# YuvalNirkin/hyperseg

Measured on AMD Instinct MI355X. Metric: frames/sec @ bs=1 HyperSeg-M 1024x512, higher is better.
Workload: dtype f32 storage and accumulation; level-4 inverted residual products as 3-term f16 splits (f32-class: 1.3e-7 of sum|a||b|; exact_f32 beside it)

## Files before the change

### hyperseg_amd/_hip.py

```python
import ctypes as C
import os

import torch

_LIB_PATH = os.environ.get('HS_HIP_LIB') or os.path.join(os.path.dirname(os.path.abspath(__file__)), 'lib',
                                                         'libhyperseg_hip.so')

ACT_NONE, ACT_RELU, ACT_RELU6, ACT_SWISH = 0, 1, 2, 3
PAD_MODES = {'zeros': 0, 'reflect': 1, 'replicate': 2, 'circular': 3}
PREV_NONE, PREV_SAME, PREV_BILINEAR = 0, 1, 2

_STATUS = {-1: 'bad argument', -2: 'feature map does not tile into the weight grid (H % fh or W % fw != 0)',
           -3: 'unsupported shape', -4: 'tile does not fit the LDS'}


class HipLibraryError(RuntimeError):
    pass


class StageInputC(C.Structure):
    _fields_ = [('skip', C.c_void_p), ('prev', C.c_void_p),
                ('batch', C.c_int32), ('H', C.c_int32), ('W', C.c_int32),
                ('c_skip', C.c_int32), ('c_prev', C.c_int32),
                ('Hp', C.c_int32), ('Wp', C.c_int32),
# ... 130 lines not shown
        'hs_mbconv_expand_dw_se_fwd': ([vp, i32, i32, i32, i32, vp, i32, vp, vp, vp, i32, i32, i32, i32, i32, i32, vp, vp, vp, C.POINTER(SeTailC), vp], C.c_int),
        'hs_se_tail_workspace': ([i32, i32, i32, i32, i64], C.c_int64),
        'hs_se_tail_tails': ([i32, i32, i32, i64], C.c_int),
        'hs_mbconv_se_workgroups': ([i32, i32, i32, i32, i32, i32], C.c_int64),
        'hs_stem_conv_fwd': ([vp, i32, i32, i32, i32, vp, i32, i32, i32, i32, i32, vp, vp, vp, vp], C.c_int),
        'hs_mbconv_tiles': ([i32, i32, i32, i32], C.c_int),
        'hs_stem_dw_fwd': ([vp, i32, i32, i32, vp, i32, vp, vp, i32, i32, i32, i32, vp, i32, i32, i32, vp, vp, vp, vp, vp], C.c_int),
        'hs_image_ingest_fwd': ([vp, i32, i32, i32, i32, i32, vp, vp, vp], C.c_int),
        'hs_stem_dw_u8_fwd': ([vp, i32, vp, i32, i32, i32, vp, i32, vp, vp, i32, i32, i32, i32, vp, i32, i32, i32, vp, vp, vp, vp, vp], C.c_int),
        'hs_overlay_fwd': ([vp, vp, i32, i32, i32, i32, vp, i32, i32, vp, vp], C.c_int),
        'hs_upsample_overlay_fwd': ([vp, i32, i32, i32, i32, i32, i32, vp, i32, vp, i32, i32, vp, vp, vp], C.c_int),
        'hs_mbconv_expand_dw_fwd': ([vp, i32, i32, i32, i32, vp, i32, vp, vp, vp, i32, i32, i32, i32, i32, i32, vp, vp, vp, vp, vp], C.c_int),
        'hs_se_gate_fwd': ([vp, i32, i32, i32, C.c_float, vp, vp, i32, vp, vp, vp, vp, vp, i32, vp, vp, vp], C.c_int),
        'hs_gemm_split_kp': ([i32], C.c_int),
        'hs_gemm_split_fwd': ([vp, vp, vp, vp, vp, i32, vp, vp, i32, i32, i32, i32, i32, vp], C.c_int),
        'hs_gemm_split_conv2x2_fwd': ([vp, vp, vp, vp, i32, vp, vp, i32, i32, i32, i32, i32, i32, vp], C.c_int),
        'hs_gemm_split_up2_fwd': ([vp, vp, vp, vp, i32, vp, i32, i32, i32, i32, i32, i32, vp], C.c_int),
        'hs_pooled_shift_fwd': ([vp, i32, C.c_float, vp, vp, vp, i32, i32, vp], C.c_int),
    }
    for name, (argtypes, restype) in sig.items():
        fn = getattr(lib, name)
        fn.argtypes, fn.restype = argtypes, restype
    if lib.hs_version() != 1:
        raise HipLibraryError(f'ABI mismatch: library reports version {lib.hs_version()}, binding expects 1')
    return lib


lib = _load()
EXPORTS = ['hs_version', 'hs_build_info', 'hs_signal2weights_fwd', 'hs_signal2weights_multi_fwd', 'hs_s2w_pack_floats', 'hs_s2w_pack_fwd', 'hs_bank_pack_fwd', 'hs_bn_fold_fwd',
           'hs_patch_conv_fwd', 'hs_patch_conv_s2w_fwd', 'hs_k1_chain_workspace', 'hs_k1_chain_fwd', 'hs_decoder_chain_workspace', 'hs_decoder_chain_fwd', 'hs_meta_conv_fwd', 'hs_meta_conv_bwd', 'hs_patch_conv_gen_fwd', 'hs_patch_ir_fwd', 'hs_patch_ir_v0_fwd', 'hs_patch_ir_v0_ws_fwd', 'hs_patch_ir_v0_workspace', 'hs_patch_ir_route', 'hs_ir_tile_map', 'hs_upsample_bilinear_fwd', 'hs_upsample_argmax_fwd',
           'hs_stage_input_fwd', 'hs_depthwise_conv_fwd', 'hs_depthwise_pool_blocks', 'hs_stem_conv_fwd', 'hs_stem_dw_fwd', 'hs_mbconv_tiles', 'hs_mbconv_expand_dw_fwd', 'hs_se_gate_fwd', 'hs_depthwise_conv_se_fwd', 'hs_mbconv_expand_dw_se_fwd', 'hs_se_tail_workspace', 'hs_se_tail_tails', 'hs_mbconv_se_workgroups', 'hs_pointwise_conv_fwd', 'hs_affine_act_fwd', 'hs_gemm_split_kp', 'hs_gemm_split_fwd', 'hs_gemm_split_conv2x2_fwd', 'hs_gemm_split_up2_fwd', 'hs_pooled_shift_fwd', 'hs_patch_conv_bwd_input',
           'hs_patch_conv_bwd_weight', 'hs_halo_tiles_fwd', 'hs_halo_tiles_bwd', 'hs_tile_interior_fwd', 'hs_tile_interior_bwd', 'hs_dw_tiles_fwd', 'hs_dw_tiles_bwd_in', 'hs_dw_tiles_bwd_w',
           'hs_s2w_train_fwd', 'hs_s2w_train_workspace', 'hs_s2w_train_bwd', 'hs_cross_entropy_fwd', 'hs_cross_entropy_bwd', 'hs_cross_entropy_typed_fwd', 'hs_cross_entropy_typed_bwd', 'hs_bootstrapped_ce_fwd', 'hs_bootstrapped_ce_bwd', 'hs_bootstrap_mean_workspace', 'hs_bootstrap_mean_fwd', 'hs_bootstrap_mean_bwd', 'hs_bootstrap_mean_batched_fwd', 'hs_bootstrap_mean_batched_bwd', 'hs_bn_train_workspace', 'hs_bn_train_stats_fwd', 'hs_dw_tiles_bn_fwd', 'hs_dw_tiles_bn_bwd_w', 'hs_patch_conv_bn_fwd', 'hs_patch_conv_bn_bwd_w', 'hs_adam_blocks', 'hs_adam_step', 'hs_bootstrap_mean_of_batch_fwd', 'hs_bootstrap_mean_of_batch_bwd', 'hs_upsample_bilinear_bwd', 'hs_upsample_bilinear_typed_bwd', 'hs_upsample_bilinear_bf16_fwd', 'hs_stage_input_typed_fwd', 'hs_bank_unpack_fwd', 'hs_bn_act_train_fwd',
           'hs_bn_act_train_bwd', 'hs_dw_tiles_bn_bwd_in_partials', 'hs_dw_tiles_bn_bwd_in', 'hs_bn_act_train_bwd_apply', 'hs_patch_conv_plain_fwd', 'hs_patch_conv_plain_bwd_in', 'hs_patch_conv_plain_bwd_w',
           'hs_upsample_bilinear_f16_fwd', 'hs_adam_step_amp', 'hs_eval_max_classes', 'hs_upsample_confusion_fwd', 'hs_confusion_fwd',
           'hs_image_ingest_fwd', 'hs_stem_dw_u8_fwd', 'hs_overlay_fwd', 'hs_upsample_overlay_fwd']


def check(status, what):
    if status == 0:
        return
    if status < 0:
        raise HipLibraryError(f'{what}: {_STATUS.get(status, status)}')
    raise HipLibraryError(f'{what}: HIP launch failed with hipError_t {status}')


# ... 35 lines not shown
```

### hyperseg_amd/csrc/hs_gemm_split.hip

```cpp
#include "hs_common.h"
#include <type_traits>

namespace hs {

using half8 = __attribute__((ext_vector_type(8))) _Float16;
using gs_f32x4 = __attribute__((ext_vector_type(4))) float;

__device__ __forceinline__ int gs_exp_of(float m) { return min(max(__float_as_int(m) >> 23, 27), 254); }
__device__ __forceinline__ float gs_scale_of(int eb) { return __int_as_float((268 - eb) << 23); }
__device__ __forceinline__ float gs_inv_scale_of(int eb) { return __int_as_float((eb - 14) << 23); }

struct GemmSplitArgs {
    const _Float16* __restrict__ wf;
    const float* __restrict__ w_inv;
    const float* __restrict__ gate; const float* __restrict__ x;
    const float* shift;
    const float* residual;
    float* y;
    int M, K, KST, N, act;
    int conv_wo;
    float* pool_partial;
    int up2_wo;
};

// ... 248 lines not shown
        ps_mean[c] = t * inv_p;
    }
    __syncthreads();
    const int r0 = 16 * blockIdx.x + 4 * wave;
    float acc[4] = {0.f, 0.f, 0.f, 0.f};
#pragma unroll 2
    for (int c = lane; c < C; c += 64) {
        const float m = ps_mean[c];
#pragma unroll
        for (int i = 0; i < 4; ++i) acc[i] = fmaf(wb[(size_t)min(r0 + i, M - 1) * C + c], m, acc[i]);
    }
#pragma unroll
    for (int i = 0; i < 4; ++i) {
        const float t = wave_sum64(acc[i]);
        if (lane == 0 && r0 + i < M) out[r0 + i] = shift[r0 + i] + t;
    }
}

static bool gemm_split_plan(int K, int& nwv, int& ks, int& nch) {
    const int steps = (K + 31) / 32;
    nwv = 2;
    while (nwv < 8 && nwv < steps) nwv *= 2;
    const int per = (steps + nwv - 1) / nwv;
    nch = per > 5 ? 2 : 1;
    ks = (steps + nwv * nch - 1) / (nwv * nch);
    return ks <= 5;
}

}

// ... 90 lines not shown
#define HS_GP(KSV, NCHV) hipLaunchKernelGGL((gemm_split_kernel<KSV, 8, true, 1, 2, NCHV, true>), grid, dim3(512), lds, s, a)
    switch (ks * 2 + nch - 1) {
        case 2: HS_GP(1, 1); break;
        case 4: HS_GP(2, 1); break;
        case 6: HS_GP(3, 1); break;
        case 8: HS_GP(4, 1); break;
        case 10: HS_GP(5, 1); break;
        case 7: HS_GP(3, 2); break;
        case 9: HS_GP(4, 2); break;
        case 11: HS_GP(5, 2); break;
        default: return HS_ERR_UNSUPPORTED;
    }
#undef HS_GP
    return launch_status();
}
```

### hyperseg_amd/functional.py

```python
import ctypes as C
import functools
import os
import threading

import torch

from . import _hip
from ._hip import ACT_NONE, ACT_RELU, ACT_RELU6, PAD_MODES

BN_EPS_DEFAULT = 1e-5
S2W_TRAIN_MAX_LAYERS = 8
COSCHEDULE_BANKS = os.environ.get('HS_COSCHEDULE_BANKS', '0') == '1'


def _round_up(n, m):
    return (n + m - 1) // m * m


def _device_of(a):
    if isinstance(a, torch.Tensor):
        return a.device
    if isinstance(a, (StageInput, BankRef, SignalRef, U8Frame)):
        return a.device
    return None
# ... 989 lines not shown
    if residual is not None and tuple(residual.shape) != shape:
        raise ValueError(f'residual has shape {tuple(residual.shape)}, expected {shape}')
    if gate is not None and tuple(gate.shape) != (b, cin):
        raise ValueError(f'gate has shape {tuple(gate.shape)}, expected {(b, cin)}')
    if shift is not None and shift.numel() != sw.c_out:
        raise ValueError(f'shift has {shift.numel()} entries, expected {sw.c_out}')
    st = _hip.lib.hs_gemm_split_fwd(_hip.dev_ptr(sw.frag, 'w_frag', torch.float16), _hip.dev_ptr(sw.inv, 'w_inv'),
                                    _hip.dev_ptr(gate, 'gate') if gate is not None else None, _hip.dev_ptr(x, 'x'),
                                    _hip.dev_ptr(shift, 'shift') if shift is not None else None, int(act),
                                    _hip.dev_ptr(residual, 'residual') if residual is not None else None,
                                    _hip.dev_ptr(out, 'out'), b, sw.c_out, cin, sw.kp, h * w, _hip.stream_ptr())
    _hip.check(st, 'hs_gemm_split_fwd')
    return out


@_on_operand_device
def gemm_split_conv2x2(sw, x, shift=None, act=ACT_NONE, out=None, pool_partial=None):
    b, cin, h, w = x.shape
    if 4 * cin != sw.c_in:
        raise ValueError(f'input has {cin} channels, the weight {sw.c_in} / 4')
    if h % 2 or w % 4:
        raise ValueError(f'map {h}x{w}: height must be even and width a multiple of 4')
    shape = (b, sw.c_out, h // 2, w // 2)
    if out is None:
        out = torch.empty(shape, device=x.device, dtype=torch.float32)
    elif tuple(out.shape) != shape:
        raise ValueError(f'out has shape {tuple(out.shape)}, expected {shape}')
    if shift is not None and shift.numel() != sw.c_out:
        raise ValueError(f'shift has {shift.numel()} entries, expected {sw.c_out}')
    nblk = -(-(h // 2) * (w // 2) // 16)
# ... 249 lines not shown
```

### hyperseg_amd/models/backbones/efficientnet.py

```python
import math
from functools import partial

import torch
import torch.nn as nn
import torch.nn.functional as F

_B0_STAGES = [
    (1, 3, 1, 32, 16, 1),
    (6, 3, 2, 16, 24, 2),
    (6, 5, 2, 24, 40, 2),
    (6, 3, 2, 40, 80, 3),
    (6, 5, 1, 80, 112, 3),
    (6, 5, 2, 112, 192, 4),
    (6, 3, 1, 192, 320, 1),
]
_SCALING = {
    'efficientnet-b0': (1.0, 1.0, 224, 0.2), 'efficientnet-b1': (1.0, 1.1, 240, 0.2),
    'efficientnet-b2': (1.1, 1.2, 260, 0.3), 'efficientnet-b3': (1.2, 1.4, 300, 0.3),
    'efficientnet-b4': (1.4, 1.8, 380, 0.4), 'efficientnet-b5': (1.6, 2.2, 456, 0.4),
    'efficientnet-b6': (1.8, 2.6, 528, 0.5), 'efficientnet-b7': (2.0, 3.1, 600, 0.5),
}
_BN_MOMENTUM, _BN_EPS, _SE_RATIO, _DIVISOR = 0.01, 1e-3, 0.25, 8


# ... 46 lines not shown
        self.stride, self.in_f, self.out_f, self.expand = stride, in_f, out_f, expand
        mid = in_f * expand
        bn = partial(nn.BatchNorm2d, momentum=_BN_MOMENTUM, eps=_BN_EPS)
        if expand != 1:
            self._expand_conv = SamePadConv2d(in_f, mid, 1, image_size=image_size, bias=False)
            self._bn0 = bn(mid)
        self._depthwise_conv = SamePadConv2d(mid, mid, kernel, stride, image_size=image_size, groups=mid, bias=False)
        self._bn1 = bn(mid)
        squeezed = max(1, int(in_f * _SE_RATIO))
        self._se_reduce = SamePadConv2d(mid, squeezed, 1, image_size=1)
        self._se_expand = SamePadConv2d(squeezed, mid, 1, image_size=1)
        self._project_conv = SamePadConv2d(mid, out_f, 1, image_size=_out_size(image_size, stride), bias=False)
        self._bn2 = bn(out_f)
        self._fused_dw = None
        self._fused_active = None

    def forward(self, inputs, drop_connect_rate=None):
        active = self._fused_active if self._fused_active is not None else _inference_only(self, inputs)
        if self._fused_dw is not None and active:
            return self._fused_dw(inputs, self)
        x = inputs
        if self.expand != 1:
            x = F.silu(self._bn0(self._expand_conv(x)))
        x = F.silu(self._bn1(self._depthwise_conv(x)))
        gate = self._se_expand(F.silu(self._se_reduce(F.adaptive_avg_pool2d(x, 1))))
        x = self._bn2(self._project_conv(torch.sigmoid(gate) * x))
        if self.stride == 1 and self.in_f == self.out_f:
            if drop_connect_rate and self.training:
                keep = 1.0 - drop_connect_rate
                mask = torch.floor(keep + torch.rand(x.shape[0], 1, 1, 1, dtype=x.dtype, device=x.device))
# ... 64 lines not shown
            return False
        h, w = (inputs.shape[2] + 1) // 2, (inputs.shape[3] + 1) // 2
        for blk in self._blocks:
            st = blk._depthwise_conv.stride[0]
            if (h * w) % 4 != 0:
                return False
            h, w = (h + st - 1) // st, (w + st - 1) // st
        return (h * w) % 4 == 0

    def takes_u8_frame(self, frame):
        f0 = self._blocks[0]._fused_dw if len(self._blocks) else None
        return self._fused_stem is not None and f0 is not None and f0.takes_image() and self._fused_ok(frame)

    def extract_features_list(self, inputs):
        use = self._fused_ok(inputs)
        for blk in self._blocks:
            blk._fused_active = use
        try:
            return self._extract_features_list(inputs, use)
        finally:
            for blk in self._blocks:
                blk._fused_active = None

    def _extract_features_list(self, inputs, use):
        f0 = self._blocks[0]._fused_dw if len(self._blocks) else None
        if self._fused_stem is not None and use and f0 is not None and getattr(f0, '_stem', None) is not None:
            x = inputs
        elif self._fused_stem is not None and use:
            x = self._fused_stem(inputs)
        else:
            x = F.silu(self._bn0(self._conv_stem(inputs)))
        feats = []
        n = len(self._blocks)
        for idx, block in enumerate(self._blocks):
            rate = self.drop_connect_rate * float(idx) / n if self.drop_connect_rate else None
            x = block(x, drop_connect_rate=rate)
            if self._res_feat_mask[idx]:
# ... 26 lines not shown
```

### hyperseg_amd/utils/inference.py

```python
import contextlib
import os

import torch
import torch.nn as nn


class InputNorm:

    LAYOUTS = ('hwc', 'chw')

    def __init__(self, mean=(0.485, 0.456, 0.406), std=(0.229, 0.224, 0.225), layout='hwc'):
        if layout not in self.LAYOUTS:
            raise ValueError(f'layout {layout!r}: expected one of {self.LAYOUTS}')
        self.mean = torch.as_tensor(mean, dtype=torch.float32).flatten().clone()
        self.std = torch.as_tensor(std, dtype=torch.float32).flatten().clone()
        if self.mean.numel() != 3 or self.std.numel() != 3:
            raise ValueError('mean and std must hold one value per channel of a 3-channel frame')
        if bool((self.std == 0).any()):
            raise ValueError('std must be non-zero')
        self.layout = layout
        values = torch.arange(256, dtype=torch.float32)
        self._tables = {torch.device('cpu'): ((values.div(255)[None, :] - self.mean[:, None]) / self.std[:, None]).contiguous()}

    def table(self, device='cpu'):
# ... 142 lines not shown
            n += 1
    return n


def _bn_affine(bn):
    with torch.no_grad():
        scale = bn.weight / torch.sqrt(bn.running_var + bn.eps)
        shift = bn.bias - bn.running_mean * scale
    return scale.detach().clone(), shift.detach().clone()


SPLIT_GEMM_MAX_K = int(os.environ.get('HS_SPLIT_GEMM_MAX_K', '1280'))
STEM_DW = os.environ.get('HS_STEM_DW', '1') != '0'
FUSE_EXPAND_MIN_PIXELS = int(os.environ.get('HS_FUSE_EXPAND_MIN_PIXELS', '2048'))
FUSE_EXPAND_MAX_CIN = int(os.environ.get('HS_FUSE_EXPAND_MAX_CIN', '40'))


LEAN_MFMA_MAX_CIN = int(os.environ.get('HS_LEAN_MFMA_MAX_CIN', '16'))
PW_MFMA_MAX_CIN = int(os.environ.get('HS_PW_MFMA_MAX_CIN', '96'))
PW_MFMA_MIN_PIXELS = int(os.environ.get('HS_PW_MFMA_MIN_PIXELS', '8192'))
GEMM_LT_MIN_PIXELS = int(os.environ.get('HS_GEMM_LT_MIN_PIXELS', '16384'))


@contextlib.contextmanager
def gemm_library(pixels, batch=1):
    want = os.environ.get('HS_BLAS') or ('cublaslt' if (pixels >= GEMM_LT_MIN_PIXELS or batch > 1) else 'cublas')
    prev = torch.backends.cuda.preferred_blas_library()
    torch.backends.cuda.preferred_blas_library(want)
    try:
        yield
# ... 48 lines not shown
        if self.split_gemm:
            sw = self.split_weights(False, x.device)
            if sw is not None:
                from .. import functional as HF
                return HF.gemm_split(sw, x.contiguous())
        with gemm_library(h * w, b):
            if b == 1:
                return torch.mm(self.conv.weight.view(-1, cin), x.view(cin, h * w)).view(1, -1, h, w)
            return torch.bmm(self.conv.weight.view(1, -1, cin).expand(b, -1, -1), x.view(b, cin, h * w)).view(b, -1, h, w)

    def forward(self, x, gate=None, residual=None):
        import torch.nn.functional as F
        from .. import functional as HF
        conv = self.conv
        x = x.contiguous()
        b, cin, h, w = x.shape
        if self.uses_mfma(x):
            return HF.pointwise_conv(x, conv.weight, gate, self.scale, self.shift, self.act, residual)
        if (h * w) % 4 != 0:
            raise NotImplementedError('feature maps with H*W % 4 != 0')
        sw = self.split_weights(True, x.device) if self.split_gemm else None
        if sw is not None:
            return HF.gemm_split(sw, x, gate=gate, shift=self.shift, act=self.act, residual=residual)
        if gate is None:
            y = F.conv2d(x, conv.weight) if b == 1 else self.raw(x)
        else:
            y = F.conv2d(x * gate[:, :, None, None], conv.weight)
        return HF.affine_act_(y, self.scale, self.shift, self.act, residual)


# ... 49 lines not shown
        self._stem = None
        if in_offset is not None:
            assert self.expand is not None, 'a depthwise conv cannot consume an offset tensor (zero padding)'
            self.expand.absorb_input_offset(in_offset)
        with torch.no_grad():
            carried = self.project.shift.clone()
            if self.skip and in_offset is not None:
                carried += in_offset.to(carried.device)
            self.defer_shift = bool(defer_shift)
            self.out_offset = carried.clone() if defer_shift else None
            self.project.shift.copy_(torch.zeros_like(carried) if defer_shift else carried)

    def takes_image(self):
        return self._stem is not None and STEM_DW

    def fuses_expand(self, x, ho, wo):
        return self.expand is not None and x.shape[1] <= FUSE_EXPAND_MAX_CIN and ho * wo >= FUSE_EXPAND_MIN_PIXELS

    def forward(self, inputs, blk):
        from .. import functional as HF
        pre = None
        if self._stem is not None and inputs.shape[1] == 3:
            stem = self._stem[0]
            img = inputs.contiguous()
            pre = HF.stem_dw(img, stem.w28, stem.scale, stem.shift, stem.pad_t, stem.pad_l, stem.out_size(img),
                             blk._depthwise_conv.weight, self.pad_t, self.pad_l, self.scale, self.shift, pool=True) if STEM_DW else None
            if pre is None and isinstance(img, HF.U8Frame):
                img = img.float_image()
            inputs = pre[0] if pre is not None else stem(img)
        x = inputs.contiguous()
        b, _, h, w = x.shape
        ho = (h + self.pad_h - self.k) // self.stride + 1
# ... 8 lines not shown
        cmid = blk._depthwise_conv.weight.shape[0]
        lean_gemm = lean and (cmid > LEAN_MFMA_MAX_CIN if self.defer_shift else not proj.mfma_covers(cmid, ho * wo))
        folds = lean_gemm and not (proj.split_gemm and proj.split_weights(True, x.device) is not None)
        se = (self._red_w, red.bias, self._exp_t, exp.bias) if self.se_tail and not folds else None
        if pre is not None:
            out = (pre[0], pre[1], False) if se is not None else pre
        elif self.fuses_expand(x, ho, wo):
            out = HF.mbconv_expand_dw(x, self.expand.conv.weight, self.expand.scale, self.expand.shift,
                                      blk._depthwise_conv.weight, self.stride, self.pad_t, self.pad_l, (ho, wo),
                                      self.scale, self.shift, pool=True, se=se)
        else:
            in_scale = in_shift = None
            if self.expand is not None:
                if lean and not self.expand.uses_mfma(x):
                    in_scale, in_shift = self.expand.scale, self.expand.shift
                    x = self.expand.raw(x)
                else:
                    x = self.expand(x)
            out = HF.depthwise_conv_bn_act(x, blk._depthwise_conv.weight, self.stride, self.pad_t, self.pad_l,
                                           (ho, wo), self.scale, self.shift, act=3, pool=True,
                                           in_scale=in_scale, in_shift=in_shift, se=se)
        y, pooled, gated = out if se is not None else (out[0], out[1], False)

        def se_gate(**fold):
            if gated and not fold:
                return pooled
            return HF.se_gate(pooled, b, ho * wo, red.weight, red.bias, self._exp_t, exp.bias, **fold)
        skip = inputs.contiguous() if self.skip else None
        if lean_gemm:
            sw = proj.split_weights(True, y.device) if proj.split_gemm else None
            if sw is not None:
                gate = se_gate()
                if self.defer_shift:
                    if skip is None:
                        return HF.gemm_split(sw, y, gate=gate)
                    return HF.gemm_split(sw, y, gate=gate, residual=skip, out=skip)
                return HF.gemm_split(sw, y, gate=gate, shift=proj.shift, residual=skip)
            wp = se_gate(w_proj=proj.conv.weight, out_scale=proj.scale)
            cmid = y.shape[1]
            with gemm_library(ho * wo, b):
                if b == 1:
                    w2d, y2d = wp.view(-1, cmid), y.view(cmid, ho * wo)
                    if self.defer_shift:
                        if skip is None:
                            return torch.mm(w2d, y2d).view(1, -1, ho, wo)
                        skip.view(-1, ho * wo).addmm_(w2d, y2d)
                        return skip
# ... 142 lines not shown
                bb._fused_fc[str(tap)] = fused
            else:
                assert offset is None
            tap += 1
    stem = bb._conv_stem
    if stem.kernel_size == (3, 3) and stem.stride == (2, 2) and stem.in_channels == 3 and isinstance(bb._bn0, nn.BatchNorm2d):
        bb._fused_stem = FusedStem(stem, bb._bn0)
        f0 = blocks[0]._fused_dw if blocks else None
        if f0 is not None and f0.expand is None and f0.k == 3 and f0.stride == 1 and not f0.skip:
            f0._stem = [bb._fused_stem]
    bb._fused_head = FusedPointwise(bb._conv_head, bb._bn1, act=3)
    if offset is not None:
        bb._fused_head.absorb_input_offset(offset)


def _install_fused(model):
    bb, wm = model.backbone, model.weight_mapper
    for blk in bb._blocks:
        blk._fused_dw = None
    bb._fused_stem = bb._fused_head = bb._fused_fc = None
    _fuse_backbone(bb)
    dev = next(model.parameters()).device
    bb.to(dev)
    if type(wm).__name__ == 'WeightMapper' and hasattr(wm, 'in_conv') and hasattr(wm, 'up_blocks') and wm.levels >= 2:
        wm._fused = FusedContextHead(wm).to(dev)
        wm._fused.split_gemm = bool(getattr(model, '_hs_split_gemm', False))
    for m in bb.modules():
        if isinstance(m, FusedPointwise):
            m.split_gemm = bool(getattr(model, '_hs_split_gemm', False))

# ... 236 lines not shown
```

### include/hyperseg_hip.h

```cpp
#ifndef HYPERSEG_HIP_H
#define HYPERSEG_HIP_H

#include <stdint.h>

#ifdef __cplusplus
extern "C" {
#endif

#define HS_ABI_VERSION 1

typedef enum {
    HS_OK = 0,
    HS_ERR_BAD_ARG = -1,
    HS_ERR_NOT_DIVISIBLE = -2,
    HS_ERR_UNSUPPORTED = -3,
    HS_ERR_LDS = -4
} hs_status;

typedef enum { HS_ACT_NONE = 0, HS_ACT_RELU = 1, HS_ACT_RELU6 = 2, HS_ACT_SWISH = 3 } hs_act;
typedef enum { HS_PAD_ZEROS = 0, HS_PAD_REFLECT = 1, HS_PAD_REPLICATE = 2, HS_PAD_CIRCULAR = 3 } hs_pad_mode;
typedef enum { HS_PREV_NONE = 0, HS_PREV_SAME = 1, HS_PREV_BILINEAR = 2 } hs_prev_mode;

typedef struct {
    const float* skip;
// ... 205 lines not shown
                               const float* w_dw, int32_t k, int32_t stride, int32_t pad_t, int32_t pad_l,
                               int32_t Ho, int32_t Wo, const float* scale1, const float* shift1, float* y,
                               const hs_se_tail* se, void* stream);

int hs_pointwise_conv_fwd(const float* x, int32_t batch, int32_t c_in, int32_t pixels, const float* w, int32_t c_out,
                          const float* gate, const float* scale, const float* shift, int32_t act, const float* residual,
                          float* y, void* stream);

int hs_affine_act_fwd(const float* x, int32_t batch, int32_t channels, int32_t pixels, const float* scale,
                      const float* shift, int32_t act, const float* residual, float* y, void* stream);

int hs_gemm_split_kp(int32_t c_in);
int hs_gemm_split_fwd(const void* w_frag, const float* w_inv, const float* gate, const float* x, const float* shift,
                      int32_t act, const float* residual, float* y, int32_t batch, int32_t c_out, int32_t c_in, int32_t kp,
                      int32_t pixels, void* stream);
int hs_gemm_split_conv2x2_fwd(const void* w_frag, const float* w_inv, const float* x, const float* shift, int32_t act, float* y,
                              float* pool_partial, int32_t batch, int32_t c_out, int32_t c_in, int32_t kp, int32_t Ho,
                              int32_t Wo, void* stream);
int hs_gemm_split_up2_fwd(const void* w_frag, const float* w_inv, const float* x, const float* shift, int32_t act, float* y,
                          int32_t batch, int32_t c_out, int32_t c_in, int32_t kp, int32_t Ho, int32_t Wo, void* stream);
int hs_pooled_shift_fwd(const float* partial, int32_t nblk, float inv_pixels, const float* wb, const float* shift,
                        float* shift_out, int32_t rows, int32_t channels, void* stream);

int hs_halo_tiles_fwd(int32_t dtype, const void* x, int32_t batch, int32_t channels, int32_t H, int32_t W, int32_t fh, int32_t fw,
                      void* tiled, int32_t patch_major, void* stream);
int hs_halo_tiles_bwd(int32_t dtype, const void* dtiled, int32_t batch, int32_t channels, int32_t H, int32_t W, int32_t fh, int32_t fw,
                      void* dx, int32_t patch_major, void* stream);
int hs_tile_interior_fwd(int32_t dtype, const void* tiled, int32_t batch, int32_t channels, int32_t H, int32_t W, int32_t fh,
                         int32_t fw, void* y, void* stream);
int hs_tile_interior_bwd(int32_t dtype, const void* dy, int32_t batch, int32_t channels, int32_t H, int32_t W, int32_t fh, int32_t fw,
// ... 102 lines not shown
```

Before: 1354.

## Fuse project GEMM with next block's expand (and decoder reducer) in one kernel

```diff
diff --git a/hyperseg_amd/_hip.py b/hyperseg_amd/_hip.py
--- a/hyperseg_amd/_hip.py
+++ b/hyperseg_amd/_hip.py
@@ -168,6 +168,8 @@
         'hs_se_gate_fwd': ([vp, i32, i32, i32, C.c_float, vp, vp, i32, vp, vp, vp, vp, vp, i32, vp, vp, vp], C.c_int),
         'hs_gemm_split_kp': ([i32], C.c_int),
         'hs_gemm_split_fwd': ([vp, vp, vp, vp, vp, i32, vp, vp, i32, i32, i32, i32, i32, vp], C.c_int),
+        'hs_gemm_split_pair_fwd': ([vp, vp, vp, vp, vp, vp, vp, i32, i32, i32, vp, vp, vp, i32, vp, i32, i32, vp, vp, vp, i32, vp, i32, i32,
+                                   i32, i32, i32, vp], C.c_int),
         'hs_gemm_split_conv2x2_fwd': ([vp, vp, vp, vp, i32, vp, vp, i32, i32, i32, i32, i32, i32, vp], C.c_int),
         'hs_gemm_split_up2_fwd': ([vp, vp, vp, vp, i32, vp, i32, i32, i32, i32, i32, i32, vp], C.c_int),
         'hs_pooled_shift_fwd': ([vp, i32, C.c_float, vp, vp, vp, i32, i32, vp], C.c_int),
@@ -183,7 +185,7 @@
 lib = _load()
 EXPORTS = ['hs_version', 'hs_build_info', 'hs_signal2weights_fwd', 'hs_signal2weights_multi_fwd', 'hs_s2w_pack_floats', 'hs_s2w_pack_fwd', 'hs_bank_pack_fwd', 'hs_bn_fold_fwd',
            'hs_patch_conv_fwd', 'hs_patch_conv_s2w_fwd', 'hs_k1_chain_workspace', 'hs_k1_chain_fwd', 'hs_decoder_chain_workspace', 'hs_decoder_chain_fwd', 'hs_meta_conv_fwd', 'hs_meta_conv_bwd', 'hs_patch_conv_gen_fwd', 'hs_patch_ir_fwd', 'hs_patch_ir_v0_fwd', 'hs_patch_ir_v0_ws_fwd', 'hs_patch_ir_v0_workspace', 'hs_patch_ir_route', 'hs_ir_tile_map', 'hs_upsample_bilinear_fwd', 'hs_upsample_argmax_fwd',
-           'hs_stage_input_fwd', 'hs_depthwise_conv_fwd', 'hs_depthwise_pool_blocks', 'hs_stem_conv_fwd', 'hs_stem_dw_fwd', 'hs_mbconv_tiles', 'hs_mbconv_expand_dw_fwd', 'hs_se_gate_fwd', 'hs_depthwise_conv_se_fwd', 'hs_mbconv_expand_dw_se_fwd', 'hs_se_tail_workspace', 'hs_se_tail_tails', 'hs_mbconv_se_workgroups', 'hs_pointwise_conv_fwd', 'hs_affine_act_fwd', 'hs_gemm_split_kp', 'hs_gemm_split_fwd', 'hs_gemm_split_conv2x2_fwd', 'hs_gemm_split_up2_fwd', 'hs_pooled_shift_fwd', 'hs_patch_conv_bwd_input',
+           'hs_stage_input_fwd', 'hs_depthwise_conv_fwd', 'hs_depthwise_pool_blocks', 'hs_stem_conv_fwd', 'hs_stem_dw_fwd', 'hs_mbconv_tiles', 'hs_mbconv_expand_dw_fwd', 'hs_se_gate_fwd', 'hs_depthwise_conv_se_fwd', 'hs_mbconv_expand_dw_se_fwd', 'hs_se_tail_workspace', 'hs_se_tail_tails', 'hs_mbconv_se_workgroups', 'hs_pointwise_conv_fwd', 'hs_affine_act_fwd', 'hs_gemm_split_kp', 'hs_gemm_split_fwd', 'hs_gemm_split_pair_fwd', 'hs_gemm_split_conv2x2_fwd', 'hs_gemm_split_up2_fwd', 'hs_pooled_shift_fwd', 'hs_patch_conv_bwd_input',
            'hs_patch_conv_bwd_weight', 'hs_halo_tiles_fwd', 'hs_halo_tiles_bwd', 'hs_tile_interior_fwd', 'hs_tile_interior_bwd', 'hs_dw_tiles_fwd', 'hs_dw_tiles_bwd_in', 'hs_dw_tiles_bwd_w',
            'hs_s2w_train_fwd', 'hs_s2w_train_workspace', 'hs_s2w_train_bwd', 'hs_cross_entropy_fwd', 'hs_cross_entropy_bwd', 'hs_cross_entropy_typed_fwd', 'hs_cross_entropy_typed_bwd', 'hs_bootstrapped_ce_fwd', 'hs_bootstrapped_ce_bwd', 'hs_bootstrap_mean_workspace', 'hs_bootstrap_mean_fwd', 'hs_bootstrap_mean_bwd', 'hs_bootstrap_mean_batched_fwd', 'hs_bootstrap_mean_batched_bwd', 'hs_bn_train_workspace', 'hs_bn_train_stats_fwd', 'hs_dw_tiles_bn_fwd', 'hs_dw_tiles_bn_bwd_w', 'hs_patch_conv_bn_fwd', 'hs_patch_conv_bn_bwd_w', 'hs_adam_blocks', 'hs_adam_step', 'hs_bootstrap_mean_of_batch_fwd', 'hs_bootstrap_mean_of_batch_bwd', 'hs_upsample_bilinear_bwd', 'hs_upsample_bilinear_typed_bwd', 'hs_upsample_bilinear_bf16_fwd', 'hs_stage_input_typed_fwd', 'hs_bank_unpack_fwd', 'hs_bn_act_train_fwd',
            'hs_bn_act_train_bwd', 'hs_dw_tiles_bn_bwd_in_partials', 'hs_dw_tiles_bn_bwd_in', 'hs_bn_act_train_bwd_apply', 'hs_patch_conv_plain_fwd', 'hs_patch_conv_plain_bwd_in', 'hs_patch_conv_plain_bwd_w',
diff --git a/hyperseg_amd/csrc/hs_gemm_split.hip b/hyperseg_amd/csrc/hs_gemm_split.hip
--- a/hyperseg_amd/csrc/hs_gemm_split.hip
+++ b/hyperseg_amd/csrc/hs_gemm_split.hip
@@ -1,5 +1,6 @@
 #include "hs_common.h"
 #include <type_traits>
+#include <algorithm>
 
 namespace hs {
 
@@ -286,6 +287,280 @@
     for (int i = 0; i < 4; ++i) {
         const float t = wave_sum64(acc[i]);
         if (lane == 0 && r0 + i < M) out[r0 + i] = shift[r0 + i] + t;
+    }
+}
+
+struct GemmPairArgs {
+    const _Float16* __restrict__ wf1; const float* __restrict__ w_inv1; const float* __restrict__ gate; const float* __restrict__ x;
+    const float* shift1; const float* residual; float* y1;
+    const _Float16* __restrict__ wf2; const float* __restrict__ w_inv2; const float* shift2; float* y2;
+    const _Float16* __restrict__ wf3; const float* __restrict__ w_inv3; const float* shift3; float* y3;
+    int M1, K1, KST1, nwv1, N, M2, KST2, act2, M3, KST3, act3;
+};
+
+__device__ __forceinline__ void gs_split8(const float* v, float sc, half8& hi, half8& lo) {
+    unsigned hh[4], ll[4];
+#pragma unroll
+    for (int j = 0; j < 4; ++j) {
+        asm("v_fma_mixlo_f16 %0, %2, %4, 0\n\t"
+            "v_fma_mixhi_f16 %0, %3, %4, 0\n\t"
+            "v_fma_mixlo_f16 %1, %2, %4, -%0 op_sel_hi:[0,0,1]\n\t"
+            "v_fma_mixhi_f16 %1, %3, %4, -%0 op_sel:[0,0,1] op_sel_hi:[0,0,1]"
+            : "=&v"(hh[j]), "=&v"(ll[j]) : "v"(v[2 * j]), "v"(v[2 * j + 1]), "v"(sc));
+    }
+    using gs_u32x4 = __attribute__((ext_vector_type(4))) unsigned;
+    hi = __builtin_bit_cast(half8, gs_u32x4{hh[0], hh[1], hh[2], hh[3]});
+    lo = __builtin_bit_cast(half8, gs_u32x4{ll[0], ll[1], ll[2], ll[3]});
+}
+
+__device__ __forceinline__ unsigned gs_colmax(unsigned mx) {
+    auto r16 = __builtin_amdgcn_permlane16_swap(mx, mx, false, false);
+    mx = max(r16[0], r16[1]);
+    auto r32 = __builtin_amdgcn_permlane32_swap(mx, mx, false, false);
+    return max(r32[0], r32[1]);
+}
+
+#ifndef HS_GP_STRIPS
+#define HS_GP_STRIPS 2
+#endif
+constexpr int GP_MAXK2 = 4;
+
+template <int KS, int NS>
+__global__ __launch_bounds__(512)
+void gemm_split_pair_kernel(GemmPairArgs a) {
+    extern __shared__ __attribute__((aligned(16))) float gp_lds[];
+    constexpr int NP = 16 * NS, PT = NP + 2 * NS, nthr = 512;
+    const int tid = threadIdx.x, lane = tid & 63, wave = tid >> 6;
+    const int lrow = lane & 15, kg = lane >> 4;
+    const int n0 = blockIdx.x * NP, b = blockIdx.z;
+    const int RT1 = (a.M1 + 15) >> 4, NR = 16 * RT1, NE = NR * NP;
+    float* tile = gp_lds;
+    float* inv2 = tile + NR * PT;
+    float* red = inv2 + GP_MAXK2 * NS * 16;
+    const float* __restrict__ xb = a.x + (size_t)b * a.K1 * a.N;
+    const float* __restrict__ gb = a.gate ? a.gate + (size_t)b * a.K1 : nullptr;
+    float* y1b = a.y1 + (size_t)b * a.M1 * a.N;
+    const float* rb = a.residual ? a.residual + (size_t)b * a.M1 * a.N : nullptr;
+    using gs_f32x2 = __attribute__((ext_vector_type(2))) float;
+
+    const int nk2 = (a.M1 + 31) >> 5;
+    const int RT2 = (a.M2 + 15) >> 4, RT3 = a.wf3 ? (a.M3 + 15) >> 4 : 0;
+    const int per = (RT2 + RT3 + gridDim.y - 1) / gridDim.y;
+    const int q1 = min(RT2 + RT3, (int)(blockIdx.y + 1) * per);
+    half8 a2h[2][GP_MAXK2], a2l[2][GP_MAXK2];
+    auto load_a2 = [&](int q, half8* h, half8* l) {
+        const bool third = q >= RT2;
+        const _Float16* wf = third ? a.wf3 : a.wf2;
+        const int rt = third ? q - RT2 : q, kst = third ? a.KST3 : a.KST2;
+#pragma unroll
+        for (int s = 0; s < GP_MAXK2; ++s)
+            if (s < nk2) {
+                const _Float16* blk = wf + ((size_t)(rt * kst + s) * 2) * 512 + lane * 8;
+                h[s] = *reinterpret_cast<const half8*>(blk);
+                l[s] = *reinterpret_cast<const half8*>(blk + 512);
+            }
+    };
+    auto load_batch = [&](int qb) {
+#pragma unroll
+        for (int u = 0; u < 2; ++u)
+            if (qb + 8 * u < q1) load_a2(qb + 8 * u, a2h[u], a2l[u]);
+    };
+    int q = blockIdx.y * per + wave;
+
+    constexpr int TE = 4 * NS;
+    float wi[TE], sh[TE], yo[TE];
+    auto load_tail = [&]() {
+#pragma unroll
+        for (int i = 0; i < TE; ++i) {
+            const int e = min(tid + i * nthr, NE - 1);
+            const int row = min(e / NP, a.M1 - 1), col = min(n0 + (e & (NP - 1)), a.N - 1);
+            wi[i] = a.w_inv1[e / NP];
+            sh[i] = a.shift1 ? a.shift1[row] : 0.0f;
+            yo[i] = rb ? rb[(size_t)row * a.N + col] : 0.0f;
+        }
+    };
+    if (wave < a.nwv1) {
+        const int ncol0 = min(n0 + NS * lrow, a.N - 1);
+        float xv[NS][KS][8];
+#pragma unroll
+        for (int s = 0; s < KS; ++s)
+#pragma unroll
+            for (int j = 0; j < 8; ++j) {
+                const int kc = min((wave * KS + s) * 32 + 8 * kg + j, a.K1 - 1);
+                if constexpr (NS == 1) {
+                    xv[0][s][j] = xb[(size_t)kc * a.N + ncol0];
+                } else {
+                    const gs_f32x2 v = *reinterpret_cast<const gs_f32x2*>(xb + (size_t)kc * a.N + ncol0);
+                    xv[0][s][j] = v[0]; xv[1][s][j] = v[1];
+                }
+            }
+        float gv[KS][8];
+#pragma unroll
+        for (int s = 0; s < KS; ++s) {
+            const int k0 = (wave * KS + s) * 32 + 8 * kg;
+            const float* gp = gb ? gb + min(k0, a.K1 - 8) : a.w_inv1;
+            const gs_f32x4 g0 = *reinterpret_cast<const gs_f32x4*>(gp), g1 = *reinterpret_cast<const gs_f32x4*>(gp + 4);
+#pragma unroll
+            for (int j = 0; j < 4; ++j) { gv[s][j] = g0[j]; gv[s][4 + j] = g1[j]; }
+        }
+        constexpr int NSL = KS <= 3 ? 3 : 2;
+        half8 ah[NSL][KS], al[NSL][KS];
+        auto load_a = [&](int rt, half8* h, half8* l) {
+#pragma unroll
+            for (int s = 0; s < KS; ++s) {
+                const _Float16* blk = a.wf1 + ((size_t)(rt * a.KST1 + wave * KS + s) * 2) * 512 + lane * 8;
+                h[s] = *reinterpret_cast<const half8*>(blk);
+                l[s] = *reinterpret_cast<const half8*>(blk + 512);
+            }
+        };
+        load_a(0, ah[0], al[0]);
+        __builtin_amdgcn_sched_barrier(0);
+        float invb[NS];
+        half8 bh[NS][KS], bl[NS][KS];
+#pragma unroll
+        for (int t = 0; t < NS; ++t) {
+            unsigned mx = 0;
+#pragma unroll
+            for (int s = 0; s < KS; ++s) {
+                const int k0 = (wave * KS + s) * 32 + 8 * kg;
+#pragma unroll
+                for (int j = 0; j < 8; ++j) {
+                    const float mk = k0 < a.K1 ? 1.0f : 0.0f;
+                    const float g = gb ? gv[s][j] * mk : mk;
+                    xv[t][s][j] *= g;
+                    mx = max(mx, __float_as_uint(xv[t][s][j]) & 0x7fffffffu);
+                }
+            }
+            const int eb = gs_exp_of(__uint_as_float(gs_colmax(mx)));
+            const float sc = gs_scale_of(eb);
+            invb[t] = gs_inv_scale_of(eb);
+#pragma unroll
+            for (int s = 0; s < KS; ++s) gs_split8(xv[t][s], sc, bh[t][s], bl[t][s]);
+        }
+        if (NSL == 3 && 1 < RT1) load_a(1, ah[1], al[1]);
+        load_tail();
+        load_batch(q);
+#pragma unroll
+        for (int mt = 0; mt < 8; ++mt) {
+            if (mt < RT1) {
+                if (mt + NSL - 1 < RT1) load_a(mt + NSL - 1, ah[(mt + NSL - 1) % NSL], al[(mt + NSL - 1) % NSL]);
+                __builtin_amdgcn_sched_barrier(0);
+#pragma unroll
+                for (int t = 0; t < NS; ++t) {
+                    gs_f32x4 acc = gs_f32x4{0.f, 0.f, 0.f, 0.f};
+#pragma unroll
+                    for (int s = 0; s < KS; ++s) {
+                        acc = __builtin_amdgcn_mfma_f32_16x16x32_f16(al[mt % NSL][s], bh[t][s], acc, 0, 0, 0);
+                        acc = __builtin_amdgcn_mfma_f32_16x16x32_f16(ah[mt % NSL][s], bl[t][s], acc, 0, 0, 0);
+                        acc = __builtin_amdgcn_mfma_f32_16x16x32_f16(ah[mt % NSL][s], bh[t][s], acc, 0, 0, 0);
+                    }
+#pragma unroll
+                    for (int r = 0; r < 4; ++r) red[(wave * NR + 16 * mt + 4 * kg + r) * NP + NS * lrow + t] = acc[r] * invb[t];
+                }
+            }
+        }
+    } else {
+        load_tail();
+        load_batch(q);
+    }
+    __syncthreads();
+#pragma unroll
+    for (int i = 0; i < TE; ++i) {
+        const int e = tid + i * nthr;
+        if (e < NE) {
+            const int row = e / NP, c = e & (NP - 1), col = n0 + c;
+            float t = 0.0f;
+#pragma unroll
+            for (int w = 0; w < 8; ++w)
+                if (w < a.nwv1) t += red[w * NE + e];
+            float v = fmaf(t, wi[i], sh[i]);
+            v += yo[i];
+            if (blockIdx.y == 0 && row < a.M1 && col < a.N) y1b[(size_t)row * a.N + col] = v;
+            tile[row * PT + c] = v;
+        }
+    }
+    __syncthreads();
+
+    _Float16* frag = reinterpret_cast<_Float16*>(red);
+    if (wave < nk2 * NS) {
+        const int s = wave / NS, t = wave - s * NS, k0 = 32 * s + 8 * kg;
+        const float mk = k0 < a.M1 ? 1.0f : 0.0f;
+        float v[8];
+        unsigned mx = 0;
+#pragma unroll
+        for (int j = 0; j < 8; ++j) {
+            v[j] = tile[min(k0 + j, a.M1 - 1) * PT + NS * lrow + t] * mk;
+            mx = max(mx, __float_as_uint(v[j]) & 0x7fffffffu);
+        }
+        const int eb = gs_exp_of(__uint_as_float(gs_colmax(mx)));
+        half8 hi, lo;
+        gs_split8(v, gs_scale_of(eb), hi, lo);
+        *reinterpret_cast<half8*>(frag + ((s * NS + t) * 2) * 512 + lane * 8) = hi;
+        *reinterpret_cast<half8*>(frag + ((s * NS + t) * 2 + 1) * 512 + lane * 8) = lo;
+        if (kg == 0) inv2[(s * NS + t) * 16 + lrow] = gs_inv_scale_of(eb);
+    }
+    __syncthreads();
+
+    half8 bh[GP_MAXK2][NS], bl[GP_MAXK2][NS];
+    float iv[GP_MAXK2][NS];
+#pragma unroll
+    for (int s = 0; s < GP_MAXK2; ++s)
+        if (s < nk2) {
+#pragma unroll
+            for (int t = 0; t < NS; ++t) {
+                bh[s][t] = *reinterpret_cast<const half8*>(frag + ((s * NS + t) * 2) * 512 + lane * 8);
+                bl[s][t] = *reinterpret_cast<const half8*>(frag + ((s * NS + t) * 2 + 1) * 512 + lane * 8);
+                iv[s][t] = inv2[(s * NS + t) * 16 + lrow];
+            }
+        }
+    for (; q < q1; q += 16) {
+#pragma unroll
+      for (int u = 0; u < 2; ++u) {
+        const int qu = q + 8 * u;
+        if (qu >= q1) break;
+        const bool third = qu >= RT2;
+        const int rt = third ? qu - RT2 : qu, M = third ? a.M3 : a.M2, act = third ? a.act3 : a.act2;
+        const float* shift = third ? a.shift3 : a.shift2;
+        float* yb = (third ? a.y3 : a.y2) + (size_t)b * M * a.N;
+        const gs_f32x4 wi4 = *reinterpret_cast<const gs_f32x4*>((third ? a.w_inv3 : a.w_inv2) + 16 * rt + 4 * kg);
+        float sh4[4];
+#pragma unroll
+        for (int r = 0; r < 4; ++r) sh4[r] = shift ? shift[min(16 * rt + 4 * kg + r, M - 1)] : 0.0f;
+        gs_f32x4 tot[NS];
+#pragma unroll
+        for (int t = 0; t < NS; ++t) {
+            tot[t] = gs_f32x4{0.f, 0.f, 0.f, 0.f};
+#pragma unroll
+            for (int s = 0; s < GP_MAXK2; ++s)
+                if (s < nk2) {
+                    gs_f32x4 acc = gs_f32x4{0.f, 0.f, 0.f, 0.f};
+                    acc = __builtin_amdgcn_mfma_f32_16x16x32_f16(a2l[u][s], bh[s][t], acc, 0, 0, 0);
+                    acc = __builtin_amdgcn_mfma_f32_16x16x32_f16(a2h[u][s], bl[s][t], acc, 0, 0, 0);
+                    acc = __builtin_amdgcn_mfma_f32_16x16x32_f16(a2h[u][s], bh[s][t], acc, 0, 0, 0);
+#pragma unroll
+                    for (int r = 0; r < 4; ++r) tot[t][r] += acc[r] * iv[s][t];
+                }
+        }
+        const int col = n0 + NS * lrow;
+#pragma unroll
+        for (int r = 0; r < 4; ++r) {
+            const int row = 16 * rt + 4 * kg + r;
+            float o[NS];
+#pragma unroll
+            for (int t = 0; t < NS; ++t) {
+                float v = fmaf(tot[t][r], wi4[r], sh4[r]);
+                if (act == HS_ACT_SWISH) v = swishf(v);
+                else if (act == HS_ACT_RELU) v = fmaxf(v, 0.0f);
+                else if (act == HS_ACT_RELU6) v = fminf(fmaxf(v, 0.0f), 6.0f);
+                o[t] = v + 0.0f;
+            }
+            if (row < M && col < a.N) {
+                if constexpr (NS == 2) *reinterpret_cast<gs_f32x2*>(yb + (size_t)row * a.N + col) = gs_f32x2{o[0], o[1]};
+                else yb[(size_t)row * a.N + col] = o[0];
+            }
+        }
+      }
+      if (q + 16 < q1) load_batch(q + 16);
     }
 }
 
@@ -406,3 +681,40 @@
 #undef HS_GP
     return launch_status();
 }
+
+extern "C" int hs_gemm_split_pair_fwd(const void* w1_frag, const float* w1_inv, const float* gate, const float* x, const float* shift1,
+                                      const float* residual, float* y1, int32_t c_mid, int32_t c_in, int32_t kp1,
+                                      const void* w2_frag, const float* w2_inv, const float* shift2, int32_t act2, float* y2, int32_t c_out2, int32_t kp2,
+                                      const void* w3_frag, const float* w3_inv, const float* shift3, int32_t act3, float* y3, int32_t c_out3, int32_t kp3,
+                                      int32_t batch, int32_t pixels, int32_t row_groups, void* stream) {
+    if (!w1_frag || !w1_inv || !x || !y1 || !w2_frag || !w2_inv || !y2 || batch <= 0 || c_mid <= 0 || c_in <= 0 || c_out2 <= 0 || pixels <= 0)
+        return HS_ERR_BAD_ARG;
+    if (act2 < 0 || act2 > 3 || row_groups < 0 || row_groups > 8) return HS_ERR_BAD_ARG;
+    if (w3_frag && (!w3_inv || !y3 || c_out3 <= 0 || act3 < 0 || act3 > 3)) return HS_ERR_BAD_ARG;
+    int nwv, ks, nch, nwv2, ks2, nch2;
+    if (!gemm_split_plan(c_in, nwv, ks, nch) || nch != 1 || ks > 4 || c_mid > 32 * GP_MAXK2) return HS_ERR_UNSUPPORTED;
+    if ((c_in & 7) || (c_mid & 7) || (pixels & 1)) return HS_ERR_UNSUPPORTED;
+    if (kp1 != nwv * ks * 32 || (ks > 1 && nwv != 8)) return HS_ERR_BAD_ARG;
+    gemm_split_plan(c_mid, nwv2, ks2, nch2);
+    if (kp2 != nwv2 * 32 || (w3_frag && kp3 != nwv2 * 32)) return HS_ERR_BAD_ARG;
+    if (batch > 65535) return HS_ERR_UNSUPPORTED;
+    const int rt23 = (c_out2 + 15) / 16 + (w3_frag ? (c_out3 + 15) / 16 : 0);
+    int rg = row_groups > 0 ? row_groups : (rt23 + 15) / 16;
+    if (residual == y1) rg = 1;
+    rg = std::min(rg, rt23);
+    GemmPairArgs a{(const _Float16*)w1_frag, w1_inv, gate, x, shift1, residual, y1,
+                   (const _Float16*)w2_frag, w2_inv, shift2, y2, (const _Float16*)w3_frag, w3_inv, shift3, y3,
+                   c_mid, c_in, kp1 / 32, nwv, pixels, c_out2, kp2 / 32, act2, c_out3, kp3 / 32, act3};
+    constexpr int NS = HS_GP_STRIPS, NP = 16 * NS;
+    const int nr = 16 * ((c_mid + 15) / 16), nk2 = (c_mid + 31) / 32;
+    const size_t lds = sizeof(float) * ((size_t)nr * (NP + 2 * NS) + GP_MAXK2 * NS * 16 + std::max(nwv * nr * NP, nk2 * NS * 512));
+    dim3 grid((pixels + NP - 1) / NP, rg, batch);
+    hipStream_t s = (hipStream_t)stream;
+#define HS_GPK(KSV) do { \
+        static std::atomic<unsigned long long> full_lds{0}; \
+        if (lds > 65536) { const int st = allow_full_lds((const void*)gemm_split_pair_kernel<KSV, NS>, full_lds); if (st != HS_OK) return st; } \
+        hipLaunchKernelGGL((gemm_split_pair_kernel<KSV, NS>), grid, dim3(512), lds, s, a); } while (0)
+    switch (ks) { case 1: HS_GPK(1); break; case 2: HS_GPK(2); break; case 3: HS_GPK(3); break; default: HS_GPK(4); break; }
+#undef HS_GPK
+    return launch_status();
+}
diff --git a/hyperseg_amd/functional.py b/hyperseg_amd/functional.py
--- a/hyperseg_amd/functional.py
+++ b/hyperseg_amd/functional.py
@@ -1027,6 +1027,48 @@
     return out
 
 
+def gemm_split_pair_covers(sw1, pixels):
+    return sw1.c_in % 8 == 0 and sw1.c_in <= 1024 and sw1.c_out % 8 == 0 and sw1.c_out <= 128 and pixels % 2 == 0
+
+
+@_on_operand_device
+def gemm_split_pair(sw1, x, sw2, gate=None, shift=None, residual=None, out=None, shift2=None, act2=ACT_NONE,
+                    sw3=None, shift3=None, act3=ACT_NONE, row_groups=0):
+    b, cin, h, w = x.shape
+    if cin != sw1.c_in:
+        raise ValueError(f'input has {cin} channels, the weight {sw1.c_in}')
+    for name, s in (('second', sw2), ('third', sw3)):
+        if s is not None and s.c_in != sw1.c_out:
+            raise ValueError(f'the {name} weight takes {s.c_in} channels, the first yields {sw1.c_out}')
+    shape = (b, sw1.c_out, h, w)
+    if out is None:
+        out = torch.empty(shape, device=x.device, dtype=torch.float32)
+    elif tuple(out.shape) != shape:
+        raise ValueError(f'out has shape {tuple(out.shape)}, expected {shape}')
+    if residual is not None and tuple(residual.shape) != shape:
+        raise ValueError(f'residual has shape {tuple(residual.shape)}, expected {shape}')
+    if gate is not None and tuple(gate.shape) != (b, cin):
+        raise ValueError(f'gate has shape {tuple(gate.shape)}, expected {(b, cin)}')
+    for name, t, s in (('shift', shift, sw1), ('shift2', shift2, sw2), ('shift3', shift3, sw3)):
+        if t is not None and (s is None or t.numel() != s.c_out):
+            raise ValueError(f'{name} has {t.numel()} entries, expected {s.c_out if s is not None else 0}')
+    y2 = torch.empty((b, sw2.c_out, h, w), device=x.device, dtype=torch.float32)
+    y3 = torch.empty((b, sw3.c_out, h, w), device=x.device, dtype=torch.float32) if sw3 is not None else None
+
+    def opt(t, name):
+        return _hip.dev_ptr(t, name) if t is not None else None
+    st = _hip.lib.hs_gemm_split_pair_fwd(
+        _hip.dev_ptr(sw1.frag, 'w1_frag', torch.float16), _hip.dev_ptr(sw1.inv, 'w1_inv'), opt(gate, 'gate'), _hip.dev_ptr(x, 'x'),
+        opt(shift, 'shift'), opt(residual, 'residual'), _hip.dev_ptr(out, 'out'), sw1.c_out, cin, sw1.kp,
+        _hip.dev_ptr(sw2.frag, 'w2_frag', torch.float16), _hip.dev_ptr(sw2.inv, 'w2_inv'), opt(shift2, 'shift2'), int(act2),
+        _hip.dev_ptr(y2, 'y2'), sw2.c_out, sw2.kp,
+        _hip.dev_ptr(sw3.frag, 'w3_frag', torch.float16) if sw3 is not None else None, opt(sw3.inv, 'w3_inv') if sw3 is not None else None,
+        opt(shift3, 'shift3'), int(act3), opt(y3, 'y3'), sw3.c_out if sw3 is not None else 0, sw3.kp if sw3 is not None else 0,
+        b, h * w, int(row_groups), _hip.stream_ptr())
+    _hip.check(st, 'hs_gemm_split_pair_fwd')
+    return (out, y2) if sw3 is None else (out, y2, y3)
+
+
 @_on_operand_device
 def gemm_split_conv2x2(sw, x, shift=None, act=ACT_NONE, out=None, pool_partial=None):
     b, cin, h, w = x.shape
diff --git a/hyperseg_amd/models/backbones/efficientnet.py b/hyperseg_amd/models/backbones/efficientnet.py
--- a/hyperseg_amd/models/backbones/efficientnet.py
+++ b/hyperseg_amd/models/backbones/efficientnet.py
@@ -84,6 +84,7 @@
         self._bn2 = bn(out_f)
         self._fused_dw = None
         self._fused_active = None
+        self._fused_after = None
 
     def forward(self, inputs, drop_connect_rate=None):
         active = self._fused_active if self._fused_active is not None else _inference_only(self, inputs)
@@ -178,13 +179,18 @@
 
     def extract_features_list(self, inputs):
         use = self._fused_ok(inputs)
-        for blk in self._blocks:
+        tap = 0
+        for idx, blk in enumerate(self._blocks):
             blk._fused_active = use
+            nxt = self._blocks[idx + 1] if idx + 1 < len(self._blocks) else None
+            fc = self._fused_fc[str(tap)] if (self._res_feat_mask[idx] and self._fused_fc is not None and str(tap) in self._fused_fc) else None
+            blk._fused_after = (nxt, fc) if use else None
+            tap += bool(self._res_feat_mask[idx])
         try:
             return self._extract_features_list(inputs, use)
         finally:
             for blk in self._blocks:
-                blk._fused_active = None
+                blk._fused_active = blk._fused_after = None
 
     def _extract_features_list(self, inputs, use):
         f0 = self._blocks[0]._fused_dw if len(self._blocks) else None
diff --git a/hyperseg_amd/utils/inference.py b/hyperseg_amd/utils/inference.py
--- a/hyperseg_amd/utils/inference.py
+++ b/hyperseg_amd/utils/inference.py
@@ -180,6 +180,13 @@
 STEM_DW = os.environ.get('HS_STEM_DW', '1') != '0'
 FUSE_EXPAND_MIN_PIXELS = int(os.environ.get('HS_FUSE_EXPAND_MIN_PIXELS', '2048'))
 FUSE_EXPAND_MAX_CIN = int(os.environ.get('HS_FUSE_EXPAND_MAX_CIN', '40'))
+GEMM_PAIR = os.environ.get('HS_GEMM_PAIR', '1') != '0'
+GEMM_PAIR_MIN_PIXELS = int(os.environ.get('HS_GEMM_PAIR_MIN_PIXELS', '2048'))
+GEMM_PAIR_MAX_PIXELS = int(os.environ.get('HS_GEMM_PAIR_MAX_PIXELS', '4608'))
+GEMM_PAIR_MIN_C = int(os.environ.get('HS_GEMM_PAIR_MIN_C', '80'))
+GEMM_PAIR_MAX_C = int(os.environ.get('HS_GEMM_PAIR_MAX_C', '128'))
+GEMM_PAIR_REDUCER = os.environ.get('HS_GEMM_PAIR_REDUCER', '1') != '0'
+GEMM_PAIR_ROW_GROUPS = int(os.environ.get('HS_GEMM_PAIR_ROW_GROUPS', '0'))
 
 
 LEAN_MFMA_MAX_CIN = int(os.environ.get('HS_LEAN_MFMA_MAX_CIN', '16'))
@@ -258,6 +265,9 @@
         from .. import functional as HF
         conv = self.conv
         x = x.contiguous()
+        made = getattr(x, '_hs_pair', None)
+        if made is not None and made.get('reduce', (None,))[0] is self and gate is None and residual is None:
+            return made['reduce'][1]
         b, cin, h, w = x.shape
         if self.uses_mfma(x):
             return HF.pointwise_conv(x, conv.weight, gate, self.scale, self.shift, self.act, residual)
@@ -337,8 +347,51 @@
     def takes_image(self):
         return self._stem is not None and STEM_DW
 
+    def pairs_with_next(self, blk, batch, ho, wo):
+        after = getattr(blk, '_fused_after', None)
+        nxt = getattr(after[0], '_fused_dw', None) if after is not None and after[0] is not None else None
+        proj = self.project
+        cout, cmid = proj.conv.weight.shape[:2]
+        pixels = ho * wo
+        if not GEMM_PAIR or not isinstance(nxt, FusedMBConv) or nxt.expand is None:
+            return None
+        if not (proj.split_gemm and cmid <= min(SPLIT_GEMM_MAX_K, 1024)):
+            return None
+        if not (cmid > LEAN_MFMA_MAX_CIN if self.defer_shift else not proj.mfma_covers(cmid, pixels)):
+            return None
+        if cmid % 8 or cout % 8 or pixels % 2 or not (GEMM_PAIR_MIN_C <= cout <= min(128, GEMM_PAIR_MAX_C)):
+            return None
+        if not (GEMM_PAIR_MIN_PIXELS <= pixels <= GEMM_PAIR_MAX_PIXELS):
+            return None
+        nho, nwo = (ho + nxt.pad_h - nxt.k) // nxt.stride + 1, (wo + nxt.pad_w - nxt.k) // nxt.stride + 1
+        if nxt._fuses_expand(cout, nho, nwo) or nxt.expand.mfma_covers(cout, pixels) or not nxt.expand.split_gemm:
+            return None
+        return nxt
+
+    def _project_pair(self, blk, nxt, sw, y, gate, skip):
+        from .. import functional as HF
+        proj = self.project
+        fc = blk._fused_after[1] if GEMM_PAIR_REDUCER else None
+        b, _, ho, wo = y.shape
+        if fc is not None and (not fc.split_gemm or fc.mfma_covers(sw.c_out, ho * wo) or (ho * wo) % 4 != 0):
+            fc = None
+        sw3 = fc.split_weights(True, y.device) if fc is not None else None
+        in_place = self.defer_shift and skip is not None and GEMM_PAIR_ROW_GROUPS == 1
+        res = HF.gemm_split_pair(sw, y, nxt.expand.split_weights(False, y.device), gate=gate,
+                                 shift=None if self.defer_shift else proj.shift, residual=skip, out=skip if in_place else None,
+                                 sw3=sw3, shift3=fc.shift if sw3 is not None else None, act3=fc.act if sw3 is not None else 0,
+                                 row_groups=GEMM_PAIR_ROW_GROUPS)
+        out = res[0]
+        out._hs_pair = {'expand': (nxt, res[1])}
+        if sw3 is not None:
+            out._hs_pair['reduce'] = (fc, res[2])
+        return out
+
+    def _fuses_expand(self, cin, ho, wo):
+        return self.expand is not None and cin <= FUSE_EXPAND_MAX_CIN and ho * wo >= FUSE_EXPAND_MIN_PIXELS
+
     def fuses_expand(self, x, ho, wo):
-        return self.expand is not None and x.shape[1] <= FUSE_EXPAND_MAX_CIN and ho * wo >= FUSE_EXPAND_MIN_PIXELS
+        return self._fuses_expand(x.shape[1], ho, wo)
 
     def forward(self, inputs, blk):
         from .. import functional as HF
@@ -377,7 +430,8 @@
             if self.expand is not None:
                 if lean and not self.expand.uses_mfma(x):
                     in_scale, in_shift = self.expand.scale, self.expand.shift
-                    x = self.expand.raw(x)
+                    made = getattr(x, '_hs_pair', None)
+                    x = made['expand'][1] if made is not None and made['expand'][0] is self else self.expand.raw(x)
                 else:
                     x = self.expand(x)
             out = HF.depthwise_conv_bn_act(x, blk._depthwise_conv.weight, self.stride, self.pad_t, self.pad_l,
@@ -394,6 +448,9 @@
             sw = proj.split_weights(True, y.device) if proj.split_gemm else None
             if sw is not None:
                 gate = se_gate()
+                nxt = self.pairs_with_next(blk, b, ho, wo)
+                if nxt is not None:
+                    return self._project_pair(blk, nxt, sw, y, gate, skip)
                 if self.defer_shift:
                     if skip is None:
                         return HF.gemm_split(sw, y, gate=gate)
@@ -566,6 +623,27 @@
         bb._fused_head.absorb_input_offset(offset)
 
 
+def pair_plan(model, height, width, batch=1):
+    bb = model.backbone
+    blocks = list(bb._blocks)
+    h, w = (height + 1) // 2, (width + 1) // 2
+    plan = []
+    for idx, blk in enumerate(blocks):
+        f = getattr(blk, '_fused_dw', None)
+        if f is None:
+            st = blk._depthwise_conv.stride[0]
+            h, w = (h + st - 1) // st, (w + st - 1) // st
+            continue
+        h, w = (h + f.pad_h - f.k) // f.stride + 1, (w + f.pad_w - f.k) // f.stride + 1
+        blk._fused_after = (blocks[idx + 1] if idx + 1 < len(blocks) else None, None)
+        try:
+            if f.pairs_with_next(blk, batch, h, w) is not None:
+                plan.append(idx)
+        finally:
+            blk._fused_after = None
+    return plan
+
+
 def _install_fused(model):
     bb, wm = model.backbone, model.weight_mapper
     for blk in bb._blocks:
diff --git a/include/hyperseg_hip.h b/include/hyperseg_hip.h
--- a/include/hyperseg_hip.h
+++ b/include/hyperseg_hip.h
@@ -243,6 +243,11 @@
 int hs_gemm_split_fwd(const void* w_frag, const float* w_inv, const float* gate, const float* x, const float* shift,
                       int32_t act, const float* residual, float* y, int32_t batch, int32_t c_out, int32_t c_in, int32_t kp,
                       int32_t pixels, void* stream);
+int hs_gemm_split_pair_fwd(const void* w1_frag, const float* w1_inv, const float* gate, const float* x, const float* shift1,
+                           const float* residual, float* y1, int32_t c_mid, int32_t c_in, int32_t kp1,
+                           const void* w2_frag, const float* w2_inv, const float* shift2, int32_t act2, float* y2, int32_t c_out2, int32_t kp2,
+                           const void* w3_frag, const float* w3_inv, const float* shift3, int32_t act3, float* y3, int32_t c_out3, int32_t kp3,
+                           int32_t batch, int32_t pixels, int32_t row_groups, void* stream);
 int hs_gemm_split_conv2x2_fwd(const void* w_frag, const float* w_inv, const float* x, const float* shift, int32_t act, float* y,
                               float* pool_partial, int32_t batch, int32_t c_out, int32_t c_in, int32_t kp, int32_t Ho,
                               int32_t Wo, void* stream);
```

New measurement: 1332. 1.6% lower.
